# allentran/golds-rl-gym

Hardware: AMD Instinct MI355X
Metric: env-steps/sec (whole node), 32k parallel Swarm-v0 envs, 20-step PAAC rollout (higher is better)
Workload: dtype f32; 1 GPU; Swarm-v0 84x84, 32768 envs per GPU, T=20 PAAC update, conv policy of train_paac_conv.py (BASELINE configs[2]); envs_per_gpu=32768, envs_total=32768, rollout_steps=20, policy=conv, train=True, swarm_math=exact, env_state_dtype=f64, streams=4, gradient_exchange=none

## Files before the change

### golds-rl-gym_amd/csrc/net_conv.hip

```cpp
#include <stdlib.h>
#include <string.h>

#include <chrono>
#include <cmath>
#include <string>
#include <vector>

#include "../../include/goldsrl_net.h"
#include "common.h"
#include "net_gemm.h"
#include "net_paac_host.h"
#include "net_reduce.inc"
#include "rng.h"

namespace grl {

enum : uint32_t { RS_ACTION = 16 };

struct ConvOffsets {
    static constexpr long c1w = 0, c1b = c1w + 8 * 8 * 3 * 32, c2w = c1b + 32, c2b = c2w + 4 * 4 * 32 * 64, c3w = c2b + 64,
                          c3b = c3w + 3 * 3 * 64 * 64, d1w = c3b + 64, d1b = d1w + 3136 * 512, d2w = d1b + 512,
                          d2b = d2w + 512 * 256, p1w = d2b + 256, p1b = p1w + 256 * 512, heads = p1b + 512;
};
constexpr int GRL_MAX_ACTIONS = 4;
// ... 47 lines not shown
    unsigned *tumask;
    unsigned *obsrec;
    unsigned *tneed2;
    float *tubias;
    float *tug, *tuspix;
    float *tslab, *tsums;
    unsigned *stmask, *szmask;
    int *sbase, *rowagent, *sblk;
    signed char *tilegroup, *org;
    signed char *ulist;
    float *slab;
    float *slab1h;
    float *slabb;
    float *slab1b;
    float *cfold;
    float *carow;
    int *cperm, *cblkcnt, *cblkoff, *cgoff, *cslot, *cinv;
    signed char *ctilegroup;
    double *slab64;
    float *ro_mu;
    float *ws_a3, *ws_d1, *ws_d2, *ws_p1, *ws_v1, *ws_v2, *ws_a3sh, *ws_d3;
    unsigned long long *ws_m3;
    unsigned long long *mb_d2, *mb_v1, *ws_mb;
    float *ws_sraw, *ws_a2sh, *ws_d2s;
    unsigned long long *ws_m2s;
    signed char *ws_ulist;
    void *ws_idx[24];
    bool train_ready;
};

struct grl_net : NetLane, grl::PaacCommNet {
    grl_net_config cfg;
    int chunk;
    float *paramsT;
    float *w3t, *w2t;
    float *w3f;
    float *wpvT;
    int shared_trunk;
    double sfrac;
    double pfrac[3];
    float *tbgimg, *tbgz, *tbgimg3, *tbgz3, *tybg;
    int *tbglist;
    int obs_index;
    int trunk_skip;
    int patch_skip;
    int gemm_f32, range_fallback_on, range_fallbacks, range_bits_last, update_skipped_last;
    int f32_by_fallback, f32_clean_passes, range_return_k, range_returns;
    float absmax_last;
    int loss_scale_on;
    int acc1;
    int expand3_gather;
    int expand2_gemm, ctiles;
    float *w2corr;
    grl::HeadOff ho;
    int npad, ptiles, pslices, pslice_rows, pwgrad_xcd, pdgrad_xcd, pwgrad_pair, pdgrad_pair, swgrad_pair, swgrad_chunks, slots_xcd;
    int tn_wgs, tn_wgs_dense;
    size_t slab_floats, slab_used, slabb_floats, slabb_used;
    std::vector<grl::RJob> rq;
    std::vector<int> rq_dst;
    int T, B;
    uint8_t *ro_lb, *ro_ab, *ro_pos, *ro_done;
    float *ro_act, *ro_envact, *ro_val, *ro_rew, *ro_y, *ro_adv, *ro_boot, *ro_pmu, *ro_psg;
    float *mu, *sigma, *vs;
    uint8_t *tmp_lb, *tmp_ab, *tmp_pos;
    int tmp_envs;
    bool prof_on;
    std::vector<hipEvent_t> prof_ev;
    std::vector<unsigned char> prof_tag;
    std::vector<double> prof_launch_flops;
    int prof_tag_cur;
    size_t prof_used;
    double prof_flops;
    int last_n;
    long ht_rollouts, ht_updates;
    double ht_rollout_ms, ht_train_enq_ms, ht_train_wait_ms;
    double ht_train_t0;
    int keep_level;
    float *keep;
    size_t keep_slots;
    long param_version, keep_version;
    int keep_max_level;
    bool keep_free_capped;
    size_t keep_free_cap, keep_headroom, keep_free_seen;
    int resident_last;
    float last_inv_total;
    NetLane lanes[GRL_MAX_LANES];
    hipStream_t lane_stream[GRL_MAX_LANES];
    hipEvent_t ev_fork, ev_join[GRL_MAX_LANES];
    hipStream_t side_stream[GRL_MAX_LANES];
    hipEvent_t ev_side0[GRL_MAX_LANES], ev_side1[GRL_MAX_LANES], ev_side2[GRL_MAX_LANES];
    int idx_side, side_now, pitem_on_side;
    int nlanes, cur_lane, last_lane;
};

namespace grl {

static void use_lane(grl_net *net, int k) {
    if (k == net->cur_lane) return;
    net->lanes[net->cur_lane] = static_cast<NetLane &>(*net);
    static_cast<NetLane &>(*net) = net->lanes[k];
    net->h->stream = net->lane_stream[k];
    net->cur_lane = k;
}
static int lanes_active(const grl_net *net) { return net->prof_on ? 1 : net->nlanes; }
static int lanes_fork(grl_net *net) {
    if (lanes_active(net) < 2) return GRL_OK;
// ... 317 lines not shown
        }
        const float zv = wave_sum(xv[r].x * wv.x + xv[r].y * wv.y + xv[r].z * wv.z + xv[r].w * wv.w);
        if (lane == 16 * r + 2 * A) mine = zv;
    }
    const int r = lane >> 4, i = lane & 15, row = row0 + r;
    if (row >= n || i > 2 * A) return;
    if (i < A) {
        mu[(size_t)row * A + i] = tanhf(mine + params[o.mub + i]);
    } else if (i < 2 * A) {
        sigma[(size_t)row * A + (i - A)] = 1.0f / (1.0f + expf(-(mine + params[o.sgb + (i - A)])));
    } else {
        const float zv = mine + params[o.v3b];
        const float sp = zv > 20.f ? zv : log1pf(expf(zv));
        vs[row] = -scale * sp;
    }
}
#define GRL_HEADS_DISPATCH(A_, CALL)                                  \
    switch (A_) {                                                     \
        case 1: { constexpr int kA = 1; CALL; } break;                \
        case 2: { constexpr int kA = 2; CALL; } break;                \
        case 3: { constexpr int kA = 3; CALL; } break;                \
        default: { constexpr int kA = 4; CALL; } break;               \
    }

struct ObsRecord {
    const uint32_t *lb, *ab, *pos;
    uint32_t *ro_lb, *ro_ab, *ro_pos;
    int nenv;
    int32_t *done_count;
};
__global__ void sample_actions_kernel(const float *__restrict__ mu, const float *__restrict__ sigma, int i0, int n, uint64_t seed,
                                      uint32_t env_off, uint32_t counter, float *__restrict__ raw, float *__restrict__ envact, ObsRecord R) {
    int i = blockIdx.x * blockDim.x + threadIdx.x;
    if (R.done_count && i == 0) *R.done_count = 0;
    for (int w = i; w < R.nenv * 50; w += gridDim.x * blockDim.x) {
        if (w < R.nenv * 40) R.ro_lb[w] = R.lb[w];
        else if (w < R.nenv * 45) R.ro_ab[w - R.nenv * 40] = R.ab[w - R.nenv * 40];
        else R.ro_pos[w - R.nenv * 45] = R.pos[w - R.nenv * 45];
    }
    if (i >= n) return;
    i += i0;
    int env = i / 10, a = i - env * 10;
    double e0, e1;
    normal_pair(rng_block(seed, (uint32_t)env + env_off, counter, RS_ACTION, a), e0, e1);
    float2 m = reinterpret_cast<const float2 *>(mu)[i], s = reinterpret_cast<const float2 *>(sigma)[i];
    float2 r = make_float2((float)((double)m.x + (double)s.x * e0), (float)((double)m.y + (double)s.y * e1));
    reinterpret_cast<float2 *>(raw)[i] = r;
    float d = sqrtf(r.x * r.x + r.y * r.y);
    if (d >= 1.0f) { r.x /= d; r.y /= d; }
    reinterpret_cast<float2 *>(envact)[i] = r;
}

#include "net_shared.inc"
#include "net_patch.inc"

#define GRL_IDX_LIST(X)                                                                                                             \
    X(perm, (size_t)net->ptiles * 256 * 4) X(sbeg, (size_t)net->pslices * 4) X(send, (size_t)net->pslices * 4)                      \
    X(sgrp, (size_t)net->pslices * 4) X(smask, c * 4) X(tmask, ((size_t)net->ptiles * 2 + 2) * 4) X(zmask, (size_t)net->pslices * 4) \
    X(tilegroup, (size_t)net->ptiles) X(org, c) X(sbase, (c + 1) * 4) X(rowagent, c * 9 * 4) X(stap, c * 9 * 2)                     \
    X(sperm, (c * 9 + 256) * 4) X(stmask, ((c * 9 + 255) / 256 + 1) * 4) X(tamask, ((c / 10) * 3 + 3) * 4)                          \
    X(tcmask, ((c / 10) * 2 + 2) * 4) X(trowlist, ((c / 10) * 81 + 256) * 4) X(tblklist, ((c / 10) * 100 + 256) * 4)               \
    X(tc3list, ((c / 10) * 49 + 256) * 4) X(trows_n, 16) X(tumask, 16)
static size_t idx_bytes_per_slot(const grl_net *net) {
    const size_t c = net->chunk;
    size_t b = 0;
#define X(m, bytes) b += ((size_t)(bytes) + 127) & ~(size_t)127;
    GRL_IDX_LIST(X)
#undef X
    return b;
}

static size_t keep_floats_per_slot(const grl_net *net, int level) {
    const size_t c = net->chunk, dense = 512 + 256 + 512 + 512 + 256 + 32;
    if (!net->shared_trunk) return c * (3136 + dense);
    size_t f = (c / 10) * 3136 + c * (1600 + 50 + dense);
    if (level >= 2) f += (c / 10) * (12800 + 5184) + c * (576 + 18) + ((c * 9 + 3) / 4 + 3) / 4 * 4;
    if (level >= 3) f = ((f + 31) & ~(size_t)31) + idx_bytes_per_slot(net) / 4;
    return f;
}

static size_t bind_activations(grl_net *net, long slot) {
    net->a3 = net->ws_a3; net->d1 = net->ws_d1; net->d2 = net->ws_d2; net->p1 = net->ws_p1; net->v1 = net->ws_v1; net->v2 = net->ws_v2;
    net->a3sh = net->ws_a3sh; net->d3 = net->ws_d3; net->m3 = net->ws_m3;
    net->mb_d2 = net->ws_mb; net->mb_v1 = net->ws_mb + (size_t)net->chunk * 4;
    net->sraw = net->ws_sraw; net->a2sh = net->ws_a2sh; net->d2s = net->ws_d2s; net->m2s = net->ws_m2s; net->ulist = net->ws_ulist;
    if (net->ws_idx[0]) {
        int k = 0;
#define X(m, bytes) net->m = static_cast<decltype(net->m)>(net->ws_idx[k++]);
        GRL_IDX_LIST(X)
#undef X
    }
    if (slot < 0 || !net->keep) return 0;
    const size_t c = net->chunk;
    float *const b0 = net->keep + (size_t)slot * keep_floats_per_slot(net, net->keep_level);
    float *b = b0;
    if (net->shared_trunk) {
        net->a3sh = b; b += (c / 10) * 3136;
        net->d3 = b; b += c * 1600;
        net->m3 = reinterpret_cast<unsigned long long *>(b); b += c * 50;
    } else {
        net->a3 = b; b += c * 3136;
    }
    net->d1 = b; b += c * 512;
    net->d2 = b; b += c * 256;
    net->p1 = b; b += c * 512;
    net->v1 = b; b += c * 512;
// ... 120 lines not shown
    n->ws_a3 = n->a3; n->ws_d1 = n->d1; n->ws_d2 = n->d2; n->ws_p1 = n->p1; n->ws_v1 = n->v1; n->ws_v2 = n->v2;
    n->ws_a3sh = n->a3sh; n->ws_d3 = n->d3; n->ws_m3 = n->m3;
    if (rc == GRL_OK) rc = paac_alloc(n, &n->ws_mb, c * 12);
    n->mb_d2 = n->ws_mb; n->mb_v1 = n->ws_mb + c * 4;
    n->ws_sraw = n->sraw; n->ws_a2sh = n->a2sh; n->ws_d2s = n->d2s; n->ws_m2s = n->m2s; n->ws_ulist = n->ulist;
    if (rc == GRL_OK) rc = paac_alloc(n, &n->perm, (size_t)n->ptiles * 256);
    if (rc == GRL_OK) rc = paac_alloc(n, &n->goffp, 32);
    if (rc == GRL_OK) rc = paac_alloc(n, &n->sbeg, n->pslices);
    if (rc == GRL_OK) rc = paac_alloc(n, &n->send, n->pslices);
    if (rc == GRL_OK) rc = paac_alloc(n, &n->sgrp, n->pslices);
    if (rc == GRL_OK) rc = paac_alloc(n, &n->blkcnt, ((c + 255) / 256) * PATCH_KEYS);
    if (rc == GRL_OK) rc = paac_alloc(n, &n->blkoff, ((c + 255) / 256) * PATCH_KEYS);
    if (rc == GRL_OK) rc = paac_alloc(n, &n->binbase, PATCH_KEYS);
    if (rc == GRL_OK) rc = paac_alloc(n, &n->pkey, c);
    if (rc == GRL_OK) rc = paac_alloc(n, &n->prank, c);
    if (rc == GRL_OK) rc = paac_alloc(n, &n->smask, c);
    if (rc == GRL_OK) rc = paac_alloc(n, &n->tmask, (size_t)n->ptiles * 2 + 2);
    if (rc == GRL_OK) rc = paac_alloc(n, &n->zmask, (size_t)n->pslices);
    if (rc == GRL_OK) rc = paac_alloc(n, &n->wmask, c);
    if (rc == GRL_OK) rc = paac_alloc(n, &n->slot_of, c);
    if (rc == GRL_OK) rc = paac_alloc(n, &n->tilegroup, (size_t)n->ptiles);
    if (rc == GRL_OK) rc = paac_alloc(n, &n->org, c);
    if (rc == GRL_OK) rc = paac_alloc(n, &n->sbase, c + 1);
    if (rc == GRL_OK) rc = paac_alloc(n, &n->rowagent, c * 9);
    if (rc == GRL_OK) rc = paac_alloc(n, &n->rowdesc, c * 9);
    if (rc == GRL_OK) rc = paac_alloc(n, &n->sblk, 1024);
    if (rc == GRL_OK) rc = paac_alloc(n, &n->skey, c * 9);
    if (rc == GRL_OK) rc = paac_alloc(n, &n->srank, c * 9);
    if (rc == GRL_OK) rc = paac_alloc(n, &n->stap, c * 9);
    if (rc == GRL_OK) rc = paac_alloc(n, &n->sblkcnt, ((c * 9 + 1023) / 1024 + 1) * 25);
    if (rc == GRL_OK) rc = paac_alloc(n, &n->sblkoff, ((c * 9 + 1023) / 1024 + 1) * 25);
    if (rc == GRL_OK) rc = paac_alloc(n, &n->sbinbase, 32);
    if (rc == GRL_OK) rc = paac_alloc(n, &n->sperm, c * 9 + 256);
    if (rc == GRL_OK) rc = paac_alloc(n, &n->stmask, (c * 9 + 255) / 256 + 1);
    if (rc == GRL_OK) rc = paac_alloc(n, &n->szmask, 1024);
    if (rc == GRL_OK) rc = paac_alloc(n, &n->tamask, (c / 10) * 3 + 3);
    if (rc == GRL_OK) rc = paac_alloc(n, &n->obsrec, (c / 10 + 1) * kObsWords);
    if (rc == GRL_OK) rc = paac_alloc(n, &n->tbmask, (c / 10) * 4 + 4);
    if (rc == GRL_OK) rc = paac_alloc(n, &n->tcmask, (c / 10) * 2 + 2);
    if (rc == GRL_OK) rc = paac_alloc(n, &n->tnmask, (c / 10) * 4 + 4);
    if (rc == GRL_OK) rc = paac_alloc(n, &n->trowlist, (c / 10) * 81 + 256);
    if (rc == GRL_OK) rc = paac_alloc(n, &n->tblklist, (c / 10) * 100 + 256);
    if (rc == GRL_OK) rc = paac_alloc(n, &n->tc3list, (c / 10) * 49 + 256);
    if (rc == GRL_OK) rc = paac_alloc(n, &n->trows_n, 4);
    if (rc == GRL_OK) rc = paac_alloc(n, &n->twgcnt, ((c / 10 + TRUNK_ENVS - 1) / TRUNK_ENVS + 1) * 3);
    if (rc == GRL_OK) rc = paac_alloc(n, &n->twgoff, ((c / 10 + TRUNK_ENVS - 1) / TRUNK_ENVS + 1) * 3);
    if (rc == GRL_OK) rc = paac_alloc(n, &n->tumask, 4);
    if (rc == GRL_OK) rc = paac_alloc(n, &n->tneed2, 4);
    if (rc == GRL_OK) rc = paac_alloc(n, &n->tubias, 512);
    if (rc == GRL_OK) rc = paac_alloc(n, &n->tug, 512);
    if (rc == GRL_OK) rc = paac_alloc(n, &n->tuspix, 49 * 64);
    if (rc == GRL_OK) rc = paac_alloc(n, &n->tslab, 2 * 2048 * 64);
    if (rc == GRL_OK) rc = paac_alloc(n, &n->tsums, 256);
    A(&n->carow, c * 128);
    if (rc == GRL_OK) rc = paac_alloc(n, &n->cperm, (size_t)n->ctiles * 256);
    if (rc == GRL_OK) rc = paac_alloc(n, &n->cblkcnt, ((c + 255) / 256) * 4);
    if (rc == GRL_OK) rc = paac_alloc(n, &n->cblkoff, ((c + 255) / 256) * 4);
    if (rc == GRL_OK) rc = paac_alloc(n, &n->cgoff, 8);
    if (rc == GRL_OK) rc = paac_alloc(n, &n->cslot, c * 9);
    if (rc == GRL_OK) rc = paac_alloc(n, &n->cinv, c);
    if (rc == GRL_OK) rc = paac_alloc(n, &n->ctilegroup, (size_t)n->ctiles);
    if (rc == GRL_OK) {
        grl_net *net = n;
        int k = 0;
#define X(m, bytes) net->ws_idx[k++] = (void *)net->m;
        GRL_IDX_LIST(X)
#undef X
        static_assert(sizeof(((NetLane *)nullptr)->ws_idx) / sizeof(void *) >= 21, "ws_idx holds every list of GRL_IDX_LIST");
    }
    return rc;
}

static int ensure_tmp_obs(grl_net *net, int n_envs) {
    if (net->tmp_envs >= n_envs) return GRL_OK;
    int rc;
    if ((rc = paac_alloc(net, &net->tmp_lb, (size_t)n_envs * 160))) return rc;
    if ((rc = paac_alloc(net, &net->tmp_ab, (size_t)n_envs * 20))) return rc;
    if ((rc = paac_alloc(net, &net->tmp_pos, (size_t)n_envs * 20))) return rc;
    float *m, *s, *v;
    if ((rc = paac_alloc(net, &m, (size_t)n_envs * 10 * net->ho.A))) return rc;
    if ((rc = paac_alloc(net, &s, (size_t)n_envs * 10 * net->ho.A))) return rc;
    if ((rc = paac_alloc(net, &v, (size_t)n_envs * 10))) return rc;
    net->mu = m; net->sigma = s; net->vs = v;
    net->tmp_envs = n_envs;
    return GRL_OK;
}

}

using namespace grl;

__global__ void grl_wait_kernel(long long ticks) {
    const long long t0 = wall_clock64();
    while (wall_clock64() - t0 < ticks) __builtin_amdgcn_s_sleep(8);
}
static int side_stream_pick(grl_net *n) {
    hipStream_t lane = n->lane_stream[0];
    hipEvent_t e0 = nullptr, e1 = nullptr, ec = nullptr;
    if (hipEventCreate(&e0) != hipSuccess || hipEventCreate(&e1) != hipSuccess || hipEventCreateWithFlags(&ec, hipEventDisableTiming) != hipSuccess) {
        (void)hipGetLastError();
        return GRL_E_HIP;
    }
    const long long ticks = 6000;
    hipStream_t cand[5] = {};
    int pick = -1;
    for (int c = 0; c < 5 && pick < 0; ++c) {
        if (hipStreamCreateWithFlags(&cand[c], hipStreamNonBlocking) != hipSuccess) { cand[c] = nullptr; break; }
// ... 51 lines not shown
    if (cfg->num_actions < 1 || cfg->num_actions > GRL_MAX_ACTIONS)
        return fail(h, GRL_E_INVALID, "grl_net_create: num_actions must be in 1..4");
    bool free_capped = false;
    unsigned long long free_mb = 0;
    if (const char *e = getenv("GRL_NET_KEEP_FREE_MB")) {
        char *end = nullptr;
        free_mb = strtoull(e, &end, 10);
        if (*e < '0' || *e > '9' || *end != 0 || free_mb >= (1ull << 44))
            return fail(h, GRL_E_INVALID, "grl_net_create: GRL_NET_KEEP_FREE_MB must be a number of MB (decimal digits)");
        free_capped = true;
    }
    hipSetDevice(h->cfg.device_id);
    grl_net *n = new grl_net();
    n->h = h; n->cfg = *cfg; n->chunk = cfg->max_chunk_samples; n->alloc_waits = true;
    n->ho = head_offsets(cfg->num_actions); n->num_params = n->ho.total;
    n->T = 0; n->B = 0; n->tmp_envs = 0; n->prof_on = false; n->prof_used = 0; n->prof_flops = 0; n->last_n = 0; n->prof_tag_cur = 0;
    n->ro_lb = nullptr; n->slab_floats = 0; n->slab_used = 0; n->slabb_floats = 0; n->slabb_used = 0; n->w3t = n->w2t = nullptr;
    n->mu = n->sigma = n->vs = nullptr;
    n->keep_level = 0;
    n->ht_rollouts = n->ht_updates = 0; n->ht_rollout_ms = n->ht_train_enq_ms = n->ht_train_wait_ms = 0.0; n->ht_train_t0 = 0.0;
    n->keep = nullptr; n->keep_slots = 0; n->param_version = 0; n->keep_version = -1;
    n->keep_max_level = 3; n->keep_free_capped = false; n->keep_free_cap = 0; n->keep_headroom = 0; n->keep_free_seen = 0;
    n->resident_last = 0;
    if (const char *e = getenv("GRL_NET_KEEP_LEVEL")) n->keep_max_level = atoi(e);
    n->keep_free_capped = free_capped; n->keep_free_cap = (size_t)free_mb << 20;
    n->shared_trunk = (cfg->reserved & GRL_NET_F_PER_AGENT_TRUNK) ? 0 : 1;
    n->cur_lane = 0; n->last_lane = 0;
    for (int k = 0; k < GRL_MAX_LANES; ++k) { n->lane_stream[k] = nullptr; n->ev_join[k] = nullptr; n->side_stream[k] = nullptr; n->ev_side0[k] = n->ev_side1[k] = n->ev_side2[k] = nullptr; }
    n->idx_side = 0; n->side_now = 0; n->pitem_on_side = 0;
    n->lane_stream[0] = h->stream; n->ev_fork = nullptr; n->nlanes = 1;
    const size_t c = n->chunk;
    n->ptiles = (int)((c + 255) / 256) + 9;
    n->ctiles = (int)((c + 255) / 256) + 4;
    {
        const char *lsk = getenv("GRL_NET_LOSS_SCALE");
        n->loss_scale_on = (lsk && strcmp(lsk, "off") == 0) ? 0 : 1;
        const char *gm = getenv("GRL_NET_GEMM"), *rf = getenv("GRL_NET_RANGE_FALLBACK");
        n->gemm_f32 = (gm && strcmp(gm, "f32") == 0) ? 1 : 0;
        n->range_fallback_on = (rf && strcmp(rf, "off") == 0) ? 0 : 1;
        n->range_fallbacks = 0; n->range_bits_last = 0; n->update_skipped_last = 0;
        n->f32_by_fallback = 0; n->f32_clean_passes = 0; n->range_returns = 0; n->absmax_last = 0.f;
        n->range_return_k = 4;
        if (const char *rr = getenv("GRL_NET_RANGE_RETURN")) n->range_return_k = strcmp(rr, "off") == 0 ? 0 : std::max(0, atoi(rr));
        const char *psk = getenv("GRL_PATCH_SKIP");
        n->patch_skip = (psk && strcmp(psk, "off") == 0) ? 0 : 1;
        const char *oix = getenv("GRL_OBS_INDEX");
        n->obs_index = (oix && strcmp(oix, "off") == 0) ? 0 : 1;
        const char *tsk = getenv("GRL_TRUNK_SKIP");
        n->trunk_skip = (tsk && strcmp(tsk, "off") == 0) ? 0 : 1;
        n->pfrac[0] = n->pfrac[1] = n->pfrac[2] = 1.0; n->sfrac = 1.0;
        const char *e2 = getenv("GRL_NET_EXPAND2");
        n->expand2_gemm = (e2 && strcmp(e2, "lds") == 0) ? 0 : 1;
        { const char *e3 = getenv("GRL_NET_EXPAND3"); n->expand3_gather = (e3 && strcmp(e3, "prod") == 0) ? 0 : 1;
          const char *a1 = getenv("GRL_NET_ACC1"); n->acc1 = (a1 && strcmp(a1, "off") == 0) ? 0 : 1; }
    }
    n->pslice_rows = PATCH_SLICE_ROWS; n->pwgrad_xcd = 1;
    if (const char *e = getenv("GRL_PATCH_SLICE")) { const int v = atoi(e); if (v == 256 || v == 512 || v == 1024 || v == 2048 || v == 4096 || v == 8192) n->pslice_rows = v; }
    if (const char *e = getenv("GRL_PATCH_WGRAD_XCD")) n->pwgrad_xcd = atoi(e);
    n->pwgrad_pair = 1;
    if (const char *e = getenv("GRL_PATCH_WGRAD_PAIR")) n->pwgrad_pair = strcmp(e, "off") != 0 && strcmp(e, "0") != 0;
    n->pdgrad_pair = 1;
    if (const char *e = getenv("GRL_PATCH_DGRAD_PAIR")) n->pdgrad_pair = strcmp(e, "off") != 0 && strcmp(e, "0") != 0;
    n->swgrad_pair = 1;
    if (const char *e = getenv("GRL_SLOT_WGRAD_PAIR")) n->swgrad_pair = strcmp(e, "off") != 0 && strcmp(e, "0") != 0;
    n->slots_xcd = 1;
    if (const char *e = getenv("GRL_SLOTS_XCD")) n->slots_xcd = strcmp(e, "off") != 0 && strcmp(e, "0") != 0;
    n->swgrad_chunks = 0;
    if (const char *e = getenv("GRL_SLOT_WGRAD_CHUNKS")) n->swgrad_chunks = std::max(0, atoi(e));
    n->pdgrad_xcd = 1;
    n->tn_wgs = 1024; n->tn_wgs_dense = 512;
    if (const char *e = getenv("GRL_TN_WGS")) { const int v = atoi(e); if (v >= 256 && v <= 4096) n->tn_wgs = v; }
    if (const char *e = getenv("GRL_TN_WGS_DENSE")) { const int v = atoi(e); if (v >= 128 && v <= 4096) n->tn_wgs_dense = v; }
    if (const char *e = getenv("GRL_PATCH_DGRAD_XCD")) n->pdgrad_xcd = atoi(e) != 0;
    n->pslices = (int)((c + n->pslice_rows - 1) / n->pslice_rows) + 9;
    n->npad = (int)((c + 255) / 256 * 256);
    int rc = GRL_OK;
    auto A = [&](float **p, size_t cnt) { if (rc == GRL_OK) rc = paac_alloc(n, p, cnt); };
    A(&n->params, n->ho.total); A(&n->paramsT, n->ho.total); A(&n->adam_m, n->ho.total); A(&n->adam_v, n->ho.total);
    A(&n->w3f, 576 * 64); A(&n->stats, 16); A(&n->wpvT, (size_t)1024 * 256); A(&n->w2corr, 4 * 576 * 128);
    A(&n->tbgimg, 12800); A(&n->tbgz, 128); A(&n->tbgimg3, 5184); A(&n->tbgz3, 128); A(&n->tybg, 49 * 512);
    if (rc == GRL_OK) rc = paac_alloc(n, &n->tbglist, 4);
    int nlanes = (cfg->reserved & GRL_NET_F_SINGLE_STREAM) ? 1 : 4;
    if (const char *env = getenv("GRL_NET_LANES")) { int v = atoi(env); if (v >= 1 && v <= GRL_MAX_LANES) nlanes = v; }
    for (int k = 0; k < nlanes && rc == GRL_OK; ++k) {
        static_cast<NetLane &>(*n) = NetLane{};
        rc = alloc_lane_forward(n);
        n->lanes[k] = static_cast<NetLane &>(*n);
    }
    static_cast<NetLane &>(*n) = n->lanes[0];
    if (rc == GRL_OK && nlanes > 1) {
        bool ok = hipEventCreateWithFlags(&n->ev_fork, hipEventDisableTiming) == hipSuccess;
        for (int k = 1; k < nlanes && ok; ++k)
            ok = hipStreamCreateWithFlags(&n->lane_stream[k], hipStreamNonBlocking) == hipSuccess &&
                 hipEventCreateWithFlags(&n->ev_join[k], hipEventDisableTiming) == hipSuccess;
        if (!ok) rc = paac_fail(n, GRL_E_HIP, "creating the lane streams/events failed");
    }
    if (rc == GRL_OK) n->nlanes = nlanes;
    {
        const char *e = getenv("GRL_NET_IDX_SIDE");
        const bool want = !(cfg->reserved & GRL_NET_F_SINGLE_STREAM) && !(e && (!strcmp(e, "off") || !strcmp(e, "0"))) && rc == GRL_OK;
        if (want && side_stream_pick(n) == GRL_OK && n->side_stream[0]) {
            const bool ok = hipEventCreateWithFlags(&n->ev_side0[0], hipEventDisableTiming) == hipSuccess &&
                            hipEventCreateWithFlags(&n->ev_side1[0], hipEventDisableTiming) == hipSuccess &&
                            hipEventCreateWithFlags(&n->ev_side2[0], hipEventDisableTiming) == hipSuccess;
            n->idx_side = ok ? 1 : 0;
        }
        (void)hipGetLastError();
// ... 362 lines not shown
```

### golds-rl-gym_amd/csrc/net_shared.inc

```

__device__ __forceinline__ bool conv1_cover(int ph, int pw, int c, int &oy1, int &ox1, int &tap1) {
    oy1 = (ph >> 2) - (c >> 1);
    ox1 = (pw >> 2) - (c & 1);
    const int ky = ph - 4 * oy1, kx = pw - 4 * ox1;
    tap1 = ky * 8 + kx;
    return oy1 >= 0 && oy1 < 20 && ox1 >= 0 && ox1 < 20;
}
__device__ __forceinline__ bool conv2_cover(int oy1, int ox1, int q, int &o2, int &tap2) {
    const int oy2 = (oy1 >> 1) - (q >> 1), ox2 = (ox1 >> 1) - (q & 1);
    tap2 = (oy1 - 2 * oy2) * 4 + (ox1 - 2 * ox2);
    o2 = oy2 * 9 + ox2;
    return oy2 >= 0 && oy2 < 9 && ox2 >= 0 && ox2 < 9;
}

__device__ __forceinline__ void agent_setup(const float *__restrict__ sraw_env, const float *__restrict__ w1, int ph, int pw, int tid,
                                            float *dlt, int *pairs, int *pix) {
    if (tid < 128) {
        const int c = tid >> 5, ci = tid & 31;
        int oy1, ox1, tap1;
        float d = 0.f;
        if (conv1_cover(ph, pw, c, oy1, ox1, tap1)) {
            const float s = sraw_env[(oy1 * 20 + ox1) * 32 + ci];
            d = fmaxf(s + w1[(tap1 * 3 + 2) * 32 + ci], 0.f) - fmaxf(s, 0.f);
        }
// ... 960 lines not shown
                       net->tubias, net->tneed2);
    PAAC_HIP(net, hipGetLastError());
    return GRL_OK;
}
static double trunk_live(grl_net *net, int which, double upper) {
    if (!net->prof_on) return upper;
    int cnt = 0;
    if (hipStreamSynchronize(net->h->stream) != hipSuccess || hipMemcpy(&cnt, net->trows_n + which, sizeof(int), hipMemcpyDeviceToHost) != hipSuccess)
        return upper;
    return (double)cnt;
}

static int trunk_background(grl_net *net) {
    if (!net->shared_trunk || !net->tbgimg) return GRL_OK;
    hipStream_t st = net->h->stream;
    const float *P = net->params, *PT = net->paramsT;
    hipLaunchKernelGGL(trunk_bg_kernel, dim3(12800 / 256), dim3(256), 0, st, P + ConvOffsets::c1b, net->tbgimg, net->tbglist);
    {
        GatherConv2ReluRows g{net->tbgimg, net->tbglist, net->tbglist + 1, net->tbgimg, 1, 1};
        EpiBiasDualRows e{nullptr, nullptr, 64, P + ConvOffsets::c2b, net->tbglist, net->tbglist + 1, net->tbgz, net->tbgz + 64};
        launch_rowk<128, 64, 4, 1, GatherConv2ReluRows, EpiBiasDualRows>(net, dim3(1, 1), st, g, PT + ConvOffsets::c2w, 512, 64, e);
    }
    hipLaunchKernelGGL(trunk_fill_kernel, dim3((81 * 16 + 255) / 256), dim3(256), 0, st, (const unsigned *)nullptr, 0, 1, (const float *)nullptr, 0,
                       (float *)nullptr, (const float *)(net->tbgz + 64), net->tbgimg3, 81, (const unsigned *)nullptr);
    {
        GatherConv3Rows g{net->tbgimg3, net->tbglist, net->tbglist + 1, net->tbgimg3, 1, 1};
        EpiBiasDualRows e{nullptr, nullptr, 64, P + ConvOffsets::c3b, net->tbglist, net->tbglist + 1, net->tbgz3, net->tbgz3 + 64};
        launch_rowk<256, 64, kW256M, kW256N, GatherConv3Rows, EpiBiasDualRows>(net, dim3(1, 1), st, g, PT + ConvOffsets::c3w, 576, 64, e);
    }
    hipLaunchKernelGGL(trunk_ybg_kernel, dim3(98), dim3(256), 0, st, (const float *)(net->tbgz3 + 64), P + ConvOffsets::d1w, net->tybg);
    PAAC_HIP(net, hipGetLastError());
    return GRL_OK;
}

static int conv1_sparse_grid() {
    int per_cu = 0, dev = 0;
    hipDeviceProp_t prop;
    if (hipOccupancyMaxActiveBlocksPerMultiprocessor(&per_cu, (const void *)conv1_sparse_shared_kernel, 256, 0) != hipSuccess || hipGetDevice(&dev) != hipSuccess ||
        hipGetDeviceProperties(&prop, dev) != hipSuccess || per_cu < 1) {
        (void)hipGetLastError();
        return 1024;
    }
    return per_cu * prop.multiProcessorCount;
}
static double trunk_union_pixels(grl_net *net) {
    if (!net->prof_on) return 49.0;
    unsigned u[2] = {0xFFFFFFFFu, 0x1FFFFu};
    if (hipStreamSynchronize(net->h->stream) == hipSuccess) (void)hipMemcpy(u, net->tumask, sizeof(u), hipMemcpyDeviceToHost);
    return (double)(__builtin_popcount(u[0]) + __builtin_popcount(u[1] & 0x1FFFFu));
}
static int patch_sort(grl_net *net, int n);
static bool pitem_gather_on(const grl_net *net);
static int pitem_index(grl_net *net, int n, const uint8_t *pos);
static int forward_conv12_shared(grl_net *net, const uint8_t *lb, const uint8_t *ab, const uint8_t *pos, int nenv, bool tail) {
    hipStream_t st = net->h->stream;
    net->pitem_on_side = 0;
    const float *P = net->params, *PT = net->paramsT;
    const int n = nenv * 10;
    const bool trunk = net->expand2_gemm && net->trunk_skip;
    const bool side = net->idx_side && net->side_now && net->cur_lane == 0 && net->expand2_gemm && !net->prof_on && net->side_stream[0];
    if (side) PAAC_HIP(net, hipEventRecord(net->ev_side0[net->cur_lane], st));
    if (trunk)
        if (int rc = trunk_index(net, lb, ab, pos, nenv)) return rc;
    if (side) PAAC_HIP(net, hipEventRecord(net->ev_side2[net->cur_lane], st));
    static const int hgc1 = conv1_sparse_grid();
    if (net->obs_index) {
        static const int hgc1i = conv1_sparse_indexed_grid();
        if (int rc = obs_index(net, lb, ab, pos, nenv, net->obsrec, st, 1)) return rc;
        hipLaunchKernelGGL(conv1_sparse_indexed_kernel, dim3(nenv < hgc1i ? nenv : hgc1i), dim3(256), 0, st, (const unsigned *)net->obsrec, P + ConvOffsets::c1w,
                           P + ConvOffsets::c1b, net->sraw, trunk ? (const unsigned *)net->tnmask : (const unsigned *)nullptr, nenv);
    } else
    hipLaunchKernelGGL(conv1_sparse_shared_kernel, dim3(nenv < hgc1 ? nenv : hgc1), dim3(256), 0, st, lb, ab, P + ConvOffsets::c1w, P + ConvOffsets::c1b,
                       net->h->cfg.grid_size, net->sraw, trunk ? (const unsigned *)net->tnmask : (const unsigned *)nullptr, nenv);
    if (trunk) {
        GatherConv2ReluRows gr{net->sraw, net->trowlist, net->trows_n, net->tbgimg, nenv * 81, 1};
        EpiBiasDualRows e{net->z2sh, net->a2sh, 64, P + ConvOffsets::c2b, net->trowlist, net->trows_n, nullptr, nullptr};
        net->prof_tag_cur = PT_ENV_FWD;
        {
            GemmTimer t(net, 2.0 * trunk_live(net, 0, (double)nenv * 81) * 512 * 64);
            launch_rowk<128, 64, 4, 1, GatherConv2ReluRows, EpiBiasDualRows>(net, dim3(1, (nenv * 81 + 127) / 128), st, gr,
                                                                                      PT + ConvOffsets::c2w, 512, 64, e);
        }
        hipLaunchKernelGGL(trunk_fill_kernel, dim3((nenv * 81 * 16 + 255) / 256), dim3(256), 0, st, (const unsigned *)net->tamask, 3, 81,
                           (const float *)(net->tbgz + 64), nenv * 81, net->a2sh, (const float *)nullptr, (float *)nullptr, 0,
                           (const unsigned *)net->tneed2);
    } else {
        GatherConv2Relu g{net->sraw, nenv * 81};
        net->prof_tag_cur = PT_ENV_FWD;
        GemmTimer t(net, 2.0 * nenv * 81 * 512 * 64);
        if (net->expand2_gemm) {
            EpiBiasDual e{net->z2sh, net->a2sh, 64, P + ConvOffsets::c2b};
            launch_rowk<256, 64, kW256M, kW256N, GatherConv2Relu, EpiBiasDual>(net, dim3(1, (nenv * 81 + 255) / 256), st, g, PT + ConvOffsets::c2w, 512, 64, e);
        } else {
            EpiBiasAct e{net->z2sh, 64, P + ConvOffsets::c2b, ACT_NONE};
            launch_rowk<256, 64, kW256M, kW256N, GatherConv2Relu, EpiBiasAct>(net, dim3(1, (nenv * 81 + 255) / 256), st, g, PT + ConvOffsets::c2w, 512, 64, e);
        }
    }
    if (side) {
        hipStream_t ss = net->side_stream[net->cur_lane];
        PAAC_HIP(net, hipStreamWaitEvent(ss, net->ev_side0[net->cur_lane], 0));
        net->h->stream = ss;
        int rc = slot_index(net, pos, n);
        if (rc == GRL_OK) {
            const int nb = (n + 255) / 256;
            hipLaunchKernelGGL(conv2_prep_kernel, dim3((n + 3) / 4), dim3(256), 0, ss, net->sraw, pos, P + ConvOffsets::c1w, net->sbase, n, net->z2sh,
                               net->carow, net->ulist, net->cslot, net->d2s, 1);
            hipLaunchKernelGGL(corr_count_kernel, dim3(nb), dim3(256), 0, ss, pos, n, net->cblkcnt);
            hipLaunchKernelGGL(corr_offsets_kernel, dim3(1), dim3(256), 0, ss, net->cblkcnt, nb, net->ctiles, net->cblkoff, net->cgoff, net->ctilegroup,
                               net->cperm);
            hipLaunchKernelGGL(corr_place_kernel, dim3(nb), dim3(256), 0, ss, pos, n, net->cblkoff, net->cgoff, net->cperm, net->cinv);
            rc = patch_sort(net, n);
            if (rc == GRL_OK && tail && pitem_gather_on(net)) {
                PAAC_HIP(net, hipStreamWaitEvent(ss, net->ev_side2[net->cur_lane], 0));
                rc = pitem_index(net, n, pos);
                net->pitem_on_side = rc == GRL_OK;
            }
        }
        net->h->stream = st;
        if (rc) return rc;
    }
    if (side) {
        PAAC_HIP(net, hipEventRecord(net->ev_side1[net->cur_lane], net->side_stream[net->cur_lane]));
        PAAC_HIP(net, hipStreamWaitEvent(st, net->ev_side1[net->cur_lane], 0));
    } else if (int rc = slot_index(net, pos, n)) return rc;
    if (net->expand2_gemm) {
        const int nb = (n + 255) / 256;
        hipLaunchKernelGGL(conv2_prep_kernel, dim3((n + 3) / 4), dim3(256), 0, st, net->sraw, pos, P + ConvOffsets::c1w, net->sbase, n, net->z2sh,
                           net->carow, net->ulist, net->cslot, net->d2s, side ? 2 : 3);
        if (!side) {
        hipLaunchKernelGGL(corr_count_kernel, dim3(nb), dim3(256), 0, st, pos, n, net->cblkcnt);
        hipLaunchKernelGGL(corr_offsets_kernel, dim3(1), dim3(256), 0, st, net->cblkcnt, nb, net->ctiles, net->cblkoff, net->cgoff, net->ctilegroup,
                           net->cperm);
        hipLaunchKernelGGL(corr_place_kernel, dim3(nb), dim3(256), 0, st, pos, n, net->cblkoff, net->cgoff, net->cperm, net->cinv);
        }
        CorrRows g{net->carow, net->cperm, net->ctilegroup, net->ctiles * 256};
        EpiConv2Corr e{net->d2s, net->m2s, net->cperm, net->cslot, net->expand3_gather && net->chunk <= (1u << 17) ? net->a2 : nullptr};
        net->prof_tag_cur = PT_CLASS_CORR;
        GemmTimer t(net, 2.0 * n * 128 * 576 * (6.25 / 9.0));
        launch_rowk<128, 64, 4, 1, CorrRows, EpiConv2Corr, true, true, 1, true>(net, dim3(576 / 64, net->ctiles * 2), st, g, net->w2corr, 128, 576, e);
    } else {
        hipLaunchKernelGGL(expand_conv2_kernel, dim3(nenv < 256 ? nenv : 256), dim3(1024), EXP2_LDS_BYTES, st, net->sraw, net->z2sh, pos,
                           P + ConvOffsets::c1w, P + ConvOffsets::c2w, nenv, net->a2sh, net->d2s, net->m2s, net->ulist, net->sbase);
    }
    PAAC_HIP(net, hipGetLastError());
    return side ? GRL_OK : patch_sort(net, n);
}

__global__ void reduce_agents_kernel(const float *__restrict__ src, int nenv, int per4, float *__restrict__ dst) {
    const size_t i = (size_t)blockIdx.x * blockDim.x + threadIdx.x;
    if (i >= (size_t)nenv * per4) return;
    const size_t e = i / per4, r = i - e * per4;
    float4 v[10];
#pragma unroll
    for (int a = 0; a < 10; ++a) v[a] = reinterpret_cast<const float4 *>(src)[(e * 10 + a) * per4 + r];
    float4 s = v[0];
#pragma unroll
    for (int a = 1; a < 10; ++a) { s.x += v[a].x; s.y += v[a].y; s.z += v[a].z; s.w += v[a].w; }
    reinterpret_cast<float4 *>(dst)[i] = s;
}

__global__ __launch_bounds__(256) void agent_dz2_kernel(const float *__restrict__ gsl, const unsigned long long *__restrict__ m2,
                                                        const float *__restrict__ a2sh, const signed char *__restrict__ ulist,
                                                        const int *__restrict__ sbase, int nenv, float *__restrict__ dz2, float *__restrict__ dza,
                                                        float *__restrict__ bsum, const unsigned *__restrict__ amask, int bgsum) {
    __shared__ __attribute__((aligned(16))) float corr[81 * 64];
    float4 cs = make_float4(0.f, 0.f, 0.f, 0.f);
    __shared__ int ul[90], sb[11], u0[10];
    __shared__ unsigned long long mw[90];
    __shared__ unsigned am[3];
    const int tid = threadIdx.x, sl = tid >> 4, c4 = (tid & 15) * 4;
    const float4 zero4 = make_float4(0.f, 0.f, 0.f, 0.f);
    for (int env = blockIdx.x; env < nenv; env += gridDim.x) {
        __syncthreads();
        for (int i = tid; i < 81 * 16; i += 256) reinterpret_cast<float4 *>(corr)[i] = zero4;
        if (tid < 11) sb[tid] = sbase[(size_t)env * 10 + tid];
        if (tid >= 64 && tid < 67) am[tid - 64] = amask ? amask[(size_t)env * 3 + tid - 64] : 0xFFFFFFFFu;
        __syncthreads();
        if (tid < 90) {
            const int a = tid / 9, j = tid - a * 9;
            const bool has = j < sb[a + 1] - sb[a];
            ul[tid] = has ? ulist[sb[a] + j] : -1;
            mw[tid] = has ? m2[(size_t)sb[a] + j] : 0ull;
        }
        float *dz = dz2 + (size_t)env * 5184;
        float4 dzv[6];
        unsigned okm = 0;
#pragma unroll
        for (int k = 0; k < 6; ++k) {
            const int i = tid + 256 * k, o = i >> 4;
            const bool ok = i < 81 * 16 && (!bgsum || ((am[o >> 5] >> (o & 31)) & 1u));
            dzv[k] = zero4;
            if (ok) dzv[k] = reinterpret_cast<const float4 *>(dz)[i];
// ... 314 lines not shown
```

Baseline: 2.264 million env-steps/s.

## Fuse conv2 correction row build into a dedicated MFMA kernel

Adds a fused conv2 correction kernel that computes the conv1-delta A rows in registers from sraw, pos and conv1 weights, instead of materialising them in a carow buffer before a generic row GEMM. The kernel streams w2corr per tap, splits it into f16 hi/lo/scaled parts in LDS, and runs a three-term split-f16 MFMA per tap with the original epilogue (d2, m2 mask, optional a2 gather, range flag). It is on by default when acc1 is set and f32 GEMM is off. It drops the carow allocation and its write and read traffic, and skips the prep kernel on the side-stream path. The cost is a more complex hand-written kernel with serialised tap loops per block.

Result: faster. 2.349 million env-steps/s, median of 6 (+3.8%).

```diff
diff --git a/golds-rl-gym_amd/csrc/net_conv.hip b/golds-rl-gym_amd/csrc/net_conv.hip
--- a/golds-rl-gym_amd/csrc/net_conv.hip
+++ b/golds-rl-gym_amd/csrc/net_conv.hip
@@ -123,6 +123,7 @@
     int expand3_gather;
     int expand2_gemm, ctiles;
     float *w2corr;
+    int corr2_fused;
     grl::HeadOff ho;
     int npad, ptiles, pslices, pslice_rows, pwgrad_xcd, pdgrad_xcd, pwgrad_pair, pdgrad_pair, swgrad_pair, swgrad_chunks, slots_xcd;
     int tn_wgs, tn_wgs_dense;
@@ -546,6 +547,7 @@
 }
 
 #include "net_shared.inc"
+#include "net_corr2.inc"
 #include "net_patch.inc"
 
 #define GRL_IDX_LIST(X)                                                                                                             \
@@ -772,7 +774,7 @@
     if (rc == GRL_OK) rc = paac_alloc(n, &n->tuspix, 49 * 64);
     if (rc == GRL_OK) rc = paac_alloc(n, &n->tslab, 2 * 2048 * 64);
     if (rc == GRL_OK) rc = paac_alloc(n, &n->tsums, 256);
-    A(&n->carow, c * 128);
+    if (!(n->corr2_fused && n->acc1 && !n->gemm_f32)) A(&n->carow, c * 128);
     if (rc == GRL_OK) rc = paac_alloc(n, &n->cperm, (size_t)n->ctiles * 256);
     if (rc == GRL_OK) rc = paac_alloc(n, &n->cblkcnt, ((c + 255) / 256) * 4);
     if (rc == GRL_OK) rc = paac_alloc(n, &n->cblkoff, ((c + 255) / 256) * 4);
@@ -930,7 +932,8 @@
         const char *e2 = getenv("GRL_NET_EXPAND2");
         n->expand2_gemm = (e2 && strcmp(e2, "lds") == 0) ? 0 : 1;
         { const char *e3 = getenv("GRL_NET_EXPAND3"); n->expand3_gather = (e3 && strcmp(e3, "prod") == 0) ? 0 : 1;
-          const char *a1 = getenv("GRL_NET_ACC1"); n->acc1 = (a1 && strcmp(a1, "off") == 0) ? 0 : 1; }
+          const char *a1 = getenv("GRL_NET_ACC1"); n->acc1 = (a1 && strcmp(a1, "off") == 0) ? 0 : 1;
+          const char *c2 = getenv("GRL_NET_CORR2"); n->corr2_fused = (c2 && strcmp(c2, "gemm") == 0) ? 0 : 1; }
     }
     n->pslice_rows = PATCH_SLICE_ROWS; n->pwgrad_xcd = 1;
     if (const char *e = getenv("GRL_PATCH_SLICE")) { const int v = atoi(e); if (v == 256 || v == 512 || v == 1024 || v == 2048 || v == 4096 || v == 8192) n->pslice_rows = v; }
diff --git a/golds-rl-gym_amd/csrc/net_corr2.inc b/golds-rl-gym_amd/csrc/net_corr2.inc
--- /dev/null
+++ b/golds-rl-gym_amd/csrc/net_corr2.inc
@@ -0,0 +1,145 @@
+__global__ __launch_bounds__(512, 4) void conv2_corr_fused_kernel(const float *__restrict__ sraw, const uint8_t *__restrict__ pos,
+                                                                  const float *__restrict__ w1, const float *__restrict__ z2sh, int zrows,
+                                                                  const int *__restrict__ perm, const signed char *__restrict__ tilegroup,
+                                                                  const int *__restrict__ cslot, const float *__restrict__ w2corr,
+                                                                  float *__restrict__ d2, unsigned long long *__restrict__ m2,
+                                                                  float *__restrict__ d2c) {
+    constexpr int LDH = kLdh, KS = 4;
+    __shared__ __attribute__((aligned(16))) unsigned short Bs[KS][3][64 * LDH];
+    const int g = tilegroup[blockIdx.x >> 1];
+    if (g < 0) return;
+    const int tid = threadIdx.x, lane = tid & 63, wave = tid >> 6, l16 = lane & 15, kg = lane >> 4;
+    const int r0 = blockIdx.x * 128 + wave * 16;
+    const int nry = 3 - (g >> 1), nrx = 3 - (g & 1);
+
+    const int trow = tid >> 3, tk4 = (tid & 7) * 4;
+    const int wo = trow * LDH + (((tk4 >> 3) ^ swz(trow)) << 3) + (tk4 & 4);
+    const float *bsrc = w2corr + ((long)g * 576 + trow) * 128 + tk4;
+    float4 rb[KS];
+#define GRL_CORR2_LOAD_B(j_) \
+    _Pragma("unroll") for (int ks = 0; ks < KS; ++ks) rb[ks] = *reinterpret_cast<const float4 *>(bsrc + (long)(j_) * 64 * 128 + ks * 32);
+    GRL_CORR2_LOAD_B(0)
+
+    int em[4], epix[4];
+#pragma unroll
+    for (int r = 0; r < 4; ++r) em[r] = perm[r0 + 4 * kg + r];
+    const int am = perm[r0 + l16];
+#pragma unroll
+    for (int r = 0; r < 4; ++r) {
+        const int m = max(em[r], 0);
+        const int ph = pos[(size_t)m * 2], pw = pos[(size_t)m * 2 + 1];
+        epix[r] = (m / 10) * 81 + ((ph >> 2) >> 1) * 9 + ((pw >> 2) >> 1);
+    }
+
+    f16x8 af[KS][2];
+    {
+        const int m = max(am, 0);
+        const int ph = pos[(size_t)m * 2], pw = pos[(size_t)m * 2 + 1];
+        const float *sraw_env = sraw + (size_t)(m / 10) * 12800;
+        float4 s[KS][2], w[KS][2];
+        bool ok[KS];
+#pragma unroll
+        for (int c = 0; c < KS; ++c) {
+            int oy1, ox1, tap1;
+            ok[c] = conv1_cover(ph, pw, c, oy1, ox1, tap1) && am >= 0;
+            const float *sp = sraw_env + (ok[c] ? (oy1 * 20 + ox1) * 32 : 0) + 8 * kg;
+            const float *wp = w1 + ((ok[c] ? tap1 : 0) * 3 + 2) * 32 + 8 * kg;
+            s[c][0] = *reinterpret_cast<const float4 *>(sp); s[c][1] = *reinterpret_cast<const float4 *>(sp + 4);
+            w[c][0] = *reinterpret_cast<const float4 *>(wp); w[c][1] = *reinterpret_cast<const float4 *>(wp + 4);
+        }
+#pragma unroll
+        for (int c = 0; c < KS; ++c) {
+            uint2 h[2], l[2];
+#pragma unroll
+            for (int q = 0; q < 2; ++q) {
+                const float4 sv = s[c][q], wv = w[c][q];
+                float4 d;
+                d.x = ok[c] ? fmaxf(sv.x + wv.x, 0.f) - fmaxf(sv.x, 0.f) : 0.f;
+                d.y = ok[c] ? fmaxf(sv.y + wv.y, 0.f) - fmaxf(sv.y, 0.f) : 0.f;
+                d.z = ok[c] ? fmaxf(sv.z + wv.z, 0.f) - fmaxf(sv.z, 0.f) : 0.f;
+                d.w = ok[c] ? fmaxf(sv.w + wv.w, 0.f) - fmaxf(sv.w, 0.f) : 0.f;
+                split4(d.x, d.y, d.z, d.w, h[q], l[q]);
+            }
+            af[c][0] = __builtin_bit_cast(f16x8, make_uint4(h[0].x, h[0].y, h[1].x, h[1].y));
+            af[c][1] = __builtin_bit_cast(f16x8, make_uint4(l[0].x, l[0].y, l[1].x, l[1].y));
+        }
+    }
+
+    const int bro = l16 * LDH + ((kg ^ swz(l16)) << 3);
+    bool out_of_range = false;
+    for (int ry = 0, rx = 0; ry < nry;) {
+        const int j = ry * 3 + rx;
+        const int rxn = rx + 1 < nrx ? rx + 1 : 0, ryn = ry + (rxn == 0);
+        int slot[4];
+        float z[4][4];
+#pragma unroll
+        for (int r = 0; r < 4; ++r) slot[r] = cslot[(size_t)max(em[r], 0) * 9 + j];
+#pragma unroll
+        for (int r = 0; r < 4; ++r) {
+            const float *zp = z2sh + (size_t)min(max(epix[r] - (ry * 9 + rx), 0), zrows - 1) * 64 + l16;
+#pragma unroll
+            for (int b = 0; b < 4; ++b) z[b][r] = zp[b * 16];
+        }
+#pragma unroll
+        for (int ks = 0; ks < KS; ++ks) {
+            uint2 h_, l_;
+            split4(rb[ks].x, rb[ks].y, rb[ks].z, rb[ks].w, h_, l_);
+            const f16x2 k_ = {(_Float16)kLowScale, (_Float16)kLowScale};
+            const f16x2 s0_ = __builtin_bit_cast(f16x2, h_.x) * k_, s1_ = __builtin_bit_cast(f16x2, h_.y) * k_;
+            *reinterpret_cast<uint2 *>(&Bs[ks][0][wo]) = h_;
+            *reinterpret_cast<uint2 *>(&Bs[ks][1][wo]) = l_;
+            *reinterpret_cast<uint2 *>(&Bs[ks][2][wo]) = make_uint2(__builtin_bit_cast(unsigned, s0_), __builtin_bit_cast(unsigned, s1_));
+        }
+        __syncthreads();
+        {
+            const int jn = ryn < nry ? ryn * 3 + rxn : j;
+            GRL_CORR2_LOAD_B(jn)
+        }
+        GRL_SCHED_FENCE
+        f32x4 acc[4];
+#pragma unroll
+        for (int b = 0; b < 4; ++b) acc[b] = f32x4{0.f, 0.f, 0.f, 0.f};
+#pragma unroll
+        for (int ks = 0; ks < KS; ++ks)
+#pragma unroll
+            for (int b = 0; b < 4; ++b) {
+                f16x8 bf[3];
+#pragma unroll
+                for (int p = 0; p < 3; ++p) bf[p] = *reinterpret_cast<const f16x8 *>(&Bs[ks][p][bro + b * 16 * LDH]);
+                acc[b] = __builtin_amdgcn_mfma_f32_16x16x32_f16(af[ks][1], bf[0], acc[b], 0, 0, 0);
+                acc[b] = __builtin_amdgcn_mfma_f32_16x16x32_f16(af[ks][0], bf[1], acc[b], 0, 0, 0);
+                acc[b] = __builtin_amdgcn_mfma_f32_16x16x32_f16(af[ks][0], bf[2], acc[b], 0, 0, 0);
+            }
+        GRL_SCHED_FENCE
+        __syncthreads();
+#pragma unroll
+        for (int r = 0; r < 4; ++r) {
+            const int sl = em[r] < 0 ? -1 : slot[r];
+            unsigned long long wbits = 0ull;
+#pragma unroll
+            for (int b = 0; b < 4; ++b) {
+                const float v = acc[b][r] * (1.0f / kLowScale);
+                const float zz = sl >= 0 ? z[b][r] : 0.f;
+                out_of_range |= !(fabsf(v + zz) <= kF16Max);
+                const unsigned long long bal = __ballot(v + zz > 0.f);
+                wbits |= ((bal >> (16 * kg)) & 0xFFFFull) << (16 * b);
+                if (sl >= 0) {
+                    const float d = fmaxf(v + zz, 0.f) - fmaxf(zz, 0.f);
+                    d2[(long)sl * 64 + b * 16 + l16] = d;
+                    if (d2c) d2c[(long)(r0 + 4 * kg + r) * 576 + j * 64 + b * 16 + l16] = d;
+                }
+            }
+            if (l16 == 0 && sl >= 0) m2[sl] = wbits;
+        }
+        ry = ryn; rx = rxn;
+    }
+#undef GRL_CORR2_LOAD_B
+    if (out_of_range) atomicOr(g_gemm_range_flag, 1);
+}
+
+static void conv2_corr_fused(grl_net *net, const uint8_t *pos, int n, hipStream_t st) {
+    hipLaunchKernelGGL(conv2_corr_fused_kernel, dim3(net->ctiles * 2), dim3(512), 0, st, (const float *)net->sraw, pos,
+                       (const float *)(net->params + ConvOffsets::c1w), (const float *)net->z2sh, (n / 10) * 81, (const int *)net->cperm,
+                       (const signed char *)net->ctilegroup, (const int *)net->cslot, (const float *)net->w2corr, net->d2s, net->m2s,
+                       net->expand3_gather && net->chunk <= (1u << 17) ? net->a2 : (float *)nullptr);
+}
diff --git a/golds-rl-gym_amd/csrc/net_shared.inc b/golds-rl-gym_amd/csrc/net_shared.inc
--- a/golds-rl-gym_amd/csrc/net_shared.inc
+++ b/golds-rl-gym_amd/csrc/net_shared.inc
@@ -1036,6 +1036,7 @@
 static int patch_sort(grl_net *net, int n);
 static bool pitem_gather_on(const grl_net *net);
 static int pitem_index(grl_net *net, int n, const uint8_t *pos);
+static void conv2_corr_fused(grl_net *net, const uint8_t *pos, int n, hipStream_t st);
 static int forward_conv12_shared(grl_net *net, const uint8_t *lb, const uint8_t *ab, const uint8_t *pos, int nenv, bool tail) {
     hipStream_t st = net->h->stream;
     net->pitem_on_side = 0;
@@ -1109,8 +1110,12 @@
     } else if (int rc = slot_index(net, pos, n)) return rc;
     if (net->expand2_gemm) {
         const int nb = (n + 255) / 256;
+        const bool fused = net->corr2_fused && net->acc1 && !net->gemm_f32;
+        if (!fused && !net->carow)
+            if (int rc = paac_alloc(net, &net->carow, (size_t)net->chunk * 128)) return rc;
+        if (!fused || !side)
         hipLaunchKernelGGL(conv2_prep_kernel, dim3((n + 3) / 4), dim3(256), 0, st, net->sraw, pos, P + ConvOffsets::c1w, net->sbase, n, net->z2sh,
-                           net->carow, net->ulist, net->cslot, net->d2s, side ? 2 : 3);
+                           net->carow, net->ulist, net->cslot, net->d2s, fused ? 1 : side ? 2 : 3);
         if (!side) {
         hipLaunchKernelGGL(corr_count_kernel, dim3(nb), dim3(256), 0, st, pos, n, net->cblkcnt);
         hipLaunchKernelGGL(corr_offsets_kernel, dim3(1), dim3(256), 0, st, net->cblkcnt, nb, net->ctiles, net->cblkoff, net->cgoff, net->ctilegroup,
@@ -1121,7 +1126,8 @@
         EpiConv2Corr e{net->d2s, net->m2s, net->cperm, net->cslot, net->expand3_gather && net->chunk <= (1u << 17) ? net->a2 : nullptr};
         net->prof_tag_cur = PT_CLASS_CORR;
         GemmTimer t(net, 2.0 * n * 128 * 576 * (6.25 / 9.0));
-        launch_rowk<128, 64, 4, 1, CorrRows, EpiConv2Corr, true, true, 1, true>(net, dim3(576 / 64, net->ctiles * 2), st, g, net->w2corr, 128, 576, e);
+        if (fused) conv2_corr_fused(net, pos, n, st);
+        else launch_rowk<128, 64, 4, 1, CorrRows, EpiConv2Corr, true, true, 1, true>(net, dim3(576 / 64, net->ctiles * 2), st, g, net->w2corr, 128, 576, e);
     } else {
         hipLaunchKernelGGL(expand_conv2_kernel, dim3(nenv < 256 ? nenv : 256), dim3(1024), EXP2_LDS_BYTES, st, net->sraw, net->z2sh, pos,
                            P + ConvOffsets::c1w, P + ConvOffsets::c2w, nenv, net->a2sh, net->d2s, net->m2s, net->ulist, net->sbase);
```
